# temudschin/xfemm

Hardware: AMD Instinct MI355X
Metric: solved DoF/s (assembly+CG to tol) on 2M-tri magnetostatic (higher is better)
Workload: dtype f64; 1 GPU; configs[2]: synthetic 2000000-tri square-domain magnetostatic, linear mu, tol 1e-08; triangles=2000000, dof_total=1002001, dof_per_gpu=1002001, nnz=7006001, pcg_iters=18, newton_iters=1, pcg=Chronopoulos-Gear + AMG V-cycle, parallelism=single GPU

## Files before the change

xfemm_amd/csrc/xfk_amg.h:

```cpp
#pragma once

#include <hip/hip_runtime.h>

#include <map>
#include <memory>
#include <vector>

#include "xfk_internal.h"
#include "xfk_partition.h"

struct xfk_comm;

namespace xfk {

constexpr int kAmgDenseMax = 2048;
constexpr int kAmgMaxLevels = 16;
constexpr int kAmgDeferSlots = 64;
constexpr int kAmgDeferTotal = kAmgDeferSlots + kAmgDeferSlots / 2;

struct AmgLevel {
    int n = 0;
    long long nnz = 0;
    int ncol_lim = 0;
    int ncol_smooth = 0;
// ... 156 lines not shown
    {
        if (side.cs) (void)hipStreamSynchronize(side.cs);
        if (sw.cs) (void)hipStreamSynchronize(sw.cs);
    }
    int setup(hipStream_t s, int n, int ncol_lim, const int *rowptr, const int *col, const double *val,
              long long nnz);
    int setup_dist(hipStream_t s, xfk_comm *comm, const HaloPlan &halo, int n, int nh, const int *rowptr,
                   const int *col, const double *val, long long nnz);
    int vcycle(hipStream_t s, const double *r, double *u, const int *done, double *part_gam = nullptr);
    bool gamma_done = false;
    int refresh(hipStream_t s, bool fold = true);
    int reserve_host();

  private:
    int init(hipStream_t s);
    int build(hipStream_t s, int l0);
    int aggregate(hipStream_t s, int l, long long &nc, bool allow_stop);
    int joins_and_p_impl(hipStream_t s, int l);
    int galerkin_dist(hipStream_t s, int l, int st, bool &rep);
    int fold_dist_tiles(hipStream_t s, int l);
    double *vc_dist(hipStream_t s, int l, const double *b, double *out, const int *done, int &rc);
    int host_ints(int count);
    int nd_order(hipStream_t s, const AmgLevel &C, int &ld);
    int resolve_deferred(hipStream_t s, bool &overflow);
    int fetch_deferred(hipStream_t s);
    int wait_deferred(hipStream_t s, bool &overflow);
    int dense_inverse(hipStream_t s, const AmgLevel &C, int ld);
    int alloc_vectors();
    int trace_strength(hipStream_t s, int l);
    int trace_aggregates(hipStream_t s, int l);
    long long ap_nnz = 0;
};

int amg_probe_info(Amg &M, hipStream_t s, xfk_amg_info *info);
int amg_probe_level_size(Amg &M, hipStream_t s, int level, int sel, int *rows, int *cols, long long *nnz);
int amg_probe_level_csr(Amg &M, hipStream_t s, int level, int sel, int *rowptr, int *col, double *val);
int amg_probe_tiles(Amg &M, hipStream_t s, int sel, int *tiles, int *wide);
int amg_probe_vector(Amg &M, hipStream_t s, int level, int what, double *out);
int amg_probe_trace(Amg &M, int level, int what, void *out);

}
```

xfemm_amd/csrc/xfk_amg.hip:

```cpp
#include <hipcub/hipcub.hpp>

#include <algorithm>
#include <climits>
#include <cmath>
#include <cstdio>
#include <cstdlib>
#include <cstring>
#include <map>
#include <mutex>
#include <vector>

#include "xfk_amg.h"
#include "xfk_comm.h"
#include "xfk_spmv.h"

namespace xfk {

namespace {


constexpr int kB = 256;
inline int nb(long long n) { return (int)((n + kB - 1) / kB); }

using MisKey = unsigned;
// ... 1014 lines not shown
    for (int s = 0; s < S; ++s) {
        bool lead = true;
#pragma unroll
        for (int q = 0; q <= s; ++q) lead = lead && !head[q];
        const double tot = lead ? cin + run[s] : run[s];
        h += head[s];
        const int nk = s + 1 < S ? key[s + 1] : __shfl_down(key[0], 1, G);
        const bool tail = key[s] != INT_MAX && (nk != key[s] || (s + 1 == S && l == G - 1));
        if (tail) {
            pcol[base + h - 1] = key[s];
            pval[base + h - 1] = tot;
        }
    }
    if (l == 0) cnt_out[row] = cnt;
}

template <int L>
__global__ void k_spgemm_compact(int nrows, int cap, const int *__restrict__ crow, const int *__restrict__ pcol,
                                 const double *__restrict__ pval, int *__restrict__ ccol, double *__restrict__ cval,
                                 int *nnz_out)
{
    const long long t = blockIdx.x * (long long)blockDim.x + threadIdx.x;
    if (t == 0 && nnz_out) *nnz_out = crow[nrows];
    const int row = (int)(t / L), l = (int)(t % L);
    if (row >= nrows) return;
    const int b = crow[row], n = crow[row + 1] - b;
    for (int m = l; m < n; m += L) {
        ccol[b + m] = pcol[(size_t)row * cap + m];
        cval[b + m] = pval[(size_t)row * cap + m];
    }
}

constexpr int kSlabLanes = 16;
__global__ void k_spgemm_compact_slab(int nrows, int nslab, int W, int stride, const int *__restrict__ crow,
                                      const int *__restrict__ slab_n, const int *__restrict__ pcol,
                                      const double *__restrict__ pval, int *__restrict__ ccol,
                                      double *__restrict__ cval, int *nnz_out)
{
    const long long t = blockIdx.x * (long long)blockDim.x + threadIdx.x;
    if (t == 0 && nnz_out) *nnz_out = crow[nrows];
    const int b = (int)(t / kSlabLanes), l = (int)(t % kSlabLanes);
    if (b >= nslab) return;
    const int d = crow[b * W], n = slab_n[b];
    const size_t src = (size_t)b * stride;
    for (int m = l; m < n; m += kSlabLanes) {
        ccol[d + m] = pcol[src + m];
        cval[d + m] = pval[src + m];
    }
}


constexpr int kBj = 64;

constexpr int kDsG = 16;
__global__ void k_dense_dscale(int n, int ld, const int *__restrict__ rowptr, const int *__restrict__ col,
                               const double *__restrict__ val, const int *__restrict__ iperm, double *__restrict__ sc)
{
    const int q = (blockIdx.x * blockDim.x + threadIdx.x) / kDsG, l = threadIdx.x % kDsG;
    if (q >= ld) return;
    const int i = iperm ? iperm[q] : (q < n ? q : -1);
    int kd = -1;
    if (i >= 0)
        for (int k = rowptr[i] + l; k < rowptr[i + 1]; k += kDsG)
            if (col[k] == i) kd = k;
#pragma unroll
    for (int off = 1; off < kDsG; off <<= 1) kd = max(kd, __shfl_xor(kd, off, kDsG));
    if (l != 0) return;
    const double d = kd >= 0 ? 0.0 + val[kd] : 0.0;
    sc[q] = d > 0.0 ? 1.0 / sqrt(d) : 1.0;
}
__global__ void k_dense_scatter(int n, int ld, const int *__restrict__ rowptr, const int *__restrict__ col,
                                const double *__restrict__ val, const int *__restrict__ perm,
                                const int *__restrict__ iperm, const double *__restrict__ sc, double *__restrict__ M)
{
    const int q = (blockIdx.x * blockDim.x + threadIdx.x) / kDsG, l = threadIdx.x % kDsG;
    if (q >= ld) return;
// ... 1139 lines not shown
    return XFK_OK;
}

int scan_only(DBuf<char> &tmp, hipStream_t s, const int *in, int *out, int n)
{
    if (n <= kScanLds) {
        k_scan_lds<<<1, 1024, 0, s>>>(n, in, out);
        AMG_CHECK(hipGetLastError());
        return XFK_OK;
    }
    size_t bytes = 0;
    AMG_CHECK(hipcub::DeviceScan::ExclusiveSum(nullptr, bytes, in, out, n + 1, s));
    AMG_CHECK(tmp.alloc(bytes ? bytes : 1));
    AMG_CHECK(hipcub::DeviceScan::ExclusiveSum(tmp.p, bytes, in, out, n + 1, s));
    return XFK_OK;
}
int scan_only(Amg &A, hipStream_t s, const int *in, int *out, int n) { return scan_only(A.cub_tmp, s, in, out, n); }

int read_flag(Amg &A, hipStream_t s, int idx, int &v)
{
    AMG_CHECK(hipMemcpyAsync(A.host_int + 1, A.dev_int.p + idx, sizeof(int), hipMemcpyDeviceToHost, s));
    AMG_CHECK(hipStreamSynchronize(s));
    v = A.host_int[1];
    return XFK_OK;
}

static bool spgemm_slab_on()
{
    return env_int("XFK_SPGEMM_SLAB", 1) != 0;
}

static int sort_rows_per_wave(int cap) { return cap == 16 ? 16 : cap <= 64 ? 8 : cap == 128 ? 4 : 2; }

void launch_compact(hipStream_t s, int nrows, int cap, const int *crow, const int *slab_n, const int *pc,
                    const double *pv, int *ccol, double *cval, int *nnz_out)
{
    if (slab_n) {
        const int W = sort_rows_per_wave(cap), nslab = (nrows + W - 1) / W;
        k_spgemm_compact_slab<<<(unsigned)(((long long)nslab * kSlabLanes + kB - 1) / kB), kB, 0, s>>>(
            nrows, nslab, W, W * cap, crow, slab_n, pc, pv, ccol, cval, nnz_out);
    } else if (cap <= 16)
        k_spgemm_compact<4><<<(unsigned)(((long long)nrows * 4 + kB - 1) / kB), kB, 0, s>>>(nrows, cap, crow, pc, pv,
                                                                                             ccol, cval, nnz_out);
    else if (cap <= 32)
        k_spgemm_compact<8><<<(unsigned)(((long long)nrows * 8 + kB - 1) / kB), kB, 0, s>>>(nrows, cap, crow, pc, pv,
                                                                                             ccol, cval, nnz_out);
    else
        k_spgemm_compact<16><<<(unsigned)(((long long)nrows * 16 + kB - 1) / kB), kB, 0, s>>>(nrows, cap, crow, pc,
                                                                                               pv, ccol, cval, nnz_out);
}

template <bool PMODE>
int spgemm(Amg &M, hipStream_t s, int nrows, const SgX &X, const SgY &Y, DBuf<int> &crow, DBuf<int> &ccol,
           DBuf<double> &cval, long long &cnnz, int key = -1, bool defer = true)
{
    AMG_CHECK(M.cnt.alloc((size_t)nrows + 1 + ((size_t)nrows + 1) / 2));
    AMG_CHECK(crow.alloc((size_t)nrows + 1));
    int *slab_n = spgemm_slab_on() ? M.cnt.p + nrows + 1 : nullptr;
    int *sovf = M.dev_int.p + 6;
    auto launch_sort = [&](int cap, int *ovf, int *need = nullptr) {
        int *pc = M.pad_col.p;
        double *pv = M.pad_val.p;
        if (nrows > 0) {
            if (cap == 16)
                k_spgemm_sort<PMODE, 4, 16><<<(nrows + 15) / 16, 64, 0, s>>>(nrows, X, Y, M.cnt.p, pc, pv, ovf, need,
                                                                             slab_n);
            else if (cap == 32)
                k_spgemm_sort<PMODE, 8, 32><<<(nrows + 7) / 8, 64, 0, s>>>(nrows, X, Y, M.cnt.p, pc, pv, ovf, need,
                                                                             slab_n);
            else if (cap == 64)
                k_spgemm_sort<PMODE, 8, 64><<<(nrows + 7) / 8, 64, 0, s>>>(nrows, X, Y, M.cnt.p, pc, pv, ovf, need,
                                                                             slab_n);
            else if (cap == 128)
                k_spgemm_sort<PMODE, 16, 128><<<(nrows + 3) / 4, 64, 0, s>>>(nrows, X, Y, M.cnt.p, pc, pv, ovf, need,
                                                                             slab_n);
            else
                k_spgemm_sort<PMODE, 32, 256><<<(nrows + 1) / 2, 64, 0, s>>>(nrows, X, Y, M.cnt.p, pc, pv, ovf, need,
                                                                             slab_n);
        }
    };
    auto sort_pass = [&](int cap, bool &overflow) -> int {
        AMG_CHECK(M.pad_col.alloc((size_t)nrows * cap));
        AMG_CHECK(M.pad_val.alloc((size_t)nrows * cap));
        AMG_CHECK(hipMemsetAsync(sovf, 0, sizeof(int), s));
        launch_sort(cap, sovf);
        AMG_CHECK(hipMemcpyAsync(M.host_int + 4, sovf, sizeof(int), hipMemcpyDeviceToHost, s));
        int rc = scan_total(M, s, M.cnt.p, crow.p, nrows, cnnz);
        if (rc != XFK_OK) return rc;
        overflow = M.host_int[4] != 0;
        if (overflow) return XFK_OK;
        AMG_CHECK(ccol.alloc((size_t)std::max(1LL, cnnz)));
        AMG_CHECK(cval.alloc((size_t)std::max(1LL, cnnz)));
        if (nrows > 0)
            launch_compact(s, nrows, cap, crow.p, slab_n, M.pad_col.p, M.pad_val.p, ccol.p, cval.p, nullptr);
        return XFK_OK;
    };
    auto deferred_pass = [&](int cap, bool verify = false) -> int {
        int *slot = M.def_dev.p + M.def_n;
        int *need = (verify && cap > 16) ? M.def_dev.p + kAmgDeferSlots + M.def_n / 2 : nullptr;
        M.def_verify[M.def_n / 2] = need ? cap : 0;
        AMG_CHECK(M.pad_col.alloc((size_t)nrows * cap));
        AMG_CHECK(M.pad_val.alloc((size_t)nrows * cap));
        AMG_CHECK(ccol.alloc((size_t)std::max(1LL, (long long)nrows * cap)));
        AMG_CHECK(cval.alloc((size_t)std::max(1LL, (long long)nrows * cap)));
        launch_sort(cap, slot, need);
        int rc = scan_only(M, s, M.cnt.p, crow.p, nrows);
        if (rc != XFK_OK) return rc;
        if (nrows > 0)
            launch_compact(s, nrows, cap, crow.p, slab_n, M.pad_col.p, M.pad_val.p, ccol.p, cval.p, slot + 1);
        else
            AMG_CHECK(hipMemsetAsync(slot + 1, 0, sizeof(int), s));
        M.def_target[M.def_n / 2] = &cnnz;
        M.def_n += 2;
        cnnz = (long long)nrows * cap;
        return XFK_OK;
    };
    if (key >= 0) {
        auto hint = M.cap_hint.find(key);
        if (hint != M.cap_hint.end()) {
            if (defer && M.def_n + 2 <= kAmgDeferSlots) return deferred_pass(hint->second, M.foreign);
            if (M.foreign) {
                M.cap_hint.erase(hint);
                hint = M.cap_hint.end();
            }
        }
        if (hint != M.cap_hint.end()) {
            bool overflow = false;
            int rc = sort_pass(hint->second, overflow);
            if (rc != XFK_OK || !overflow) return rc;
            M.cap_hint.erase(hint);
        }
    }
    int maxprod = 0;
    if (nrows > 0) {
        k_spgemm_nprod<PMODE><<<nb(nrows), kB, 0, s>>>(nrows, X, Y, M.cnt.p);
        size_t bytes = 0;
        AMG_CHECK(hipcub::DeviceReduce::Max(nullptr, bytes, M.cnt.p, M.dev_int.p + 3, nrows, s));
        AMG_CHECK(M.cub_tmp.alloc(bytes ? bytes : 1));
        AMG_CHECK(hipcub::DeviceReduce::Max(M.cub_tmp.p, bytes, M.cnt.p, M.dev_int.p + 3, nrows, s));
        int rc = read_flag(M, s, 3, maxprod);
        if (rc != XFK_OK) return rc;
    }
// ... 61 lines not shown
    const int g = (n + 255) / 256;
    if (G <= 4) {
        if (acc) k_csr_mv_tile<256, true, 2><<<g, 256, 0, s>>>(n, rowptr, col, val, x, y, done, c16, cbase);
        else k_csr_mv_tile<256, false, 2><<<g, 256, 0, s>>>(n, rowptr, col, val, x, y, done, c16, cbase);
    } else {
        if (acc) k_csr_mv_tile<256, true, 6><<<g, 256, 0, s>>>(n, rowptr, col, val, x, y, done, c16, cbase);
        else k_csr_mv_tile<256, false, 6><<<g, 256, 0, s>>>(n, rowptr, col, val, x, y, done, c16, cbase);
    }
}

void launch_mv(hipStream_t s, int n, const int *rowptr, const int *col, const double *val, const double *x, double *y,
               bool acc, int G, const int *done, const unsigned short *c16 = nullptr, const int *cbase = nullptr)
{
    if (n <= 0) return;
    if (n >= kTileMinRows && G <= 8) {
        const int g = (n + 255) / 256;
        if (G <= 4) {
            if (acc) k_csr_mv_tile<256, true, 2><<<g, 256, 0, s>>>(n, rowptr, col, val, x, y, done, c16, cbase);
            else k_csr_mv_tile<256, false, 2><<<g, 256, 0, s>>>(n, rowptr, col, val, x, y, done, c16, cbase);
        } else {
            if (acc) k_csr_mv_tile<256, true, 6><<<g, 256, 0, s>>>(n, rowptr, col, val, x, y, done, c16, cbase);
            else k_csr_mv_tile<256, false, 6><<<g, 256, 0, s>>>(n, rowptr, col, val, x, y, done, c16, cbase);
        }
        return;
    }
    const int g = (int)(((long long)n * G + 255) / 256);
#define XFK_MV(GG)                                                                                        \
    if (acc) k_csr_mv_g<GG, true><<<g, 256, 0, s>>>(n, rowptr, col, val, x, y, done);                    \
    else k_csr_mv_g<GG, false><<<g, 256, 0, s>>>(n, rowptr, col, val, x, y, done);
    if (G == 4) { XFK_MV(4) } else if (G == 8) { XFK_MV(8) } else { XFK_MV(16) }
#undef XFK_MV
}

}

__global__ void k_tile_halo_flags(int n, int B, const int *__restrict__ rowptr, const int *__restrict__ col,
                                  int *__restrict__ flag)
{
    const int i = blockIdx.x * blockDim.x + threadIdx.x;
    if (i >= n) return;
    bool h = false;
    for (int k = rowptr[i]; k < rowptr[i + 1]; ++k) h = h || col[k] >= n;
    if (h) flag[i / B] = 1;
}

int build_tile_split(hipStream_t s, int n, int B, const int *rowptr, const int *col, TileSplit &ts)
{
    const int nt = (n + B - 1) / B;
    ts.B = 0;
    ts.n_in = ts.n_bd = 0;
    if (nt == 0) {
        ts.B = B;
        return XFK_OK;
    }
    DBuf<int> flag;
    AMG_CHECK(flag.alloc(nt));
    AMG_CHECK(hipMemsetAsync(flag.p, 0, sizeof(int) * nt, s));
    k_tile_halo_flags<<<nb(n), kB, 0, s>>>(n, B, rowptr, col, flag.p);
    std::vector<int> h(nt), list;
    list.reserve(nt);
    AMG_CHECK(hipMemcpyAsync(h.data(), flag.p, sizeof(int) * nt, hipMemcpyDeviceToHost, s));
    AMG_CHECK(hipStreamSynchronize(s));
    for (int t = 0; t < nt; ++t)
        if (!h[t]) list.push_back(t);
    ts.n_in = (int)list.size();
    for (int t = 0; t < nt; ++t)
// ... 2103 lines not shown
```

xfemm_amd/csrc/xfk_api.hip:

```cpp
#include <hipcub/hipcub.hpp>

#include "xfk_amg.h"
#include "xfk_spmv.h"

#include <algorithm>
#include <atomic>
#include <chrono>
#include <cmath>
#include <cstring>
#include <map>
#include <mutex>
#include <iterator>
#include <set>
#include <type_traits>
#include <unordered_map>

#include "xfk_age.h"
#include "xfk_comm.h"
#include "xfk_kernels.h"
#include "xfk_magdir.h"
#include <cstdio>
#include <cstdlib>
#include "xfk_partition.h"

// ... 603 lines not shown

hipError_t d2h(void *dst, const void *src, size_t bytes, hipStream_t s)
{
    hipError_t e = hipMemcpyAsync(dst, src, bytes, hipMemcpyDeviceToHost, s);
    if (e != hipSuccess) return e;
    return hipStreamSynchronize(s);
}

static hipError_t cub_scratch(xfk_problem *P, size_t bytes, void **out)
{
    hipError_t e = P->cub_tmp.alloc(bytes ? bytes : 1);
    *out = P->cub_tmp.p;
    return e;
}

static hipError_t exclusive_scan(xfk_problem *P, const int *in, int *out, int n)
{
    hipStream_t s = P->stream;
    void *tmp = nullptr;
    size_t bytes = 0;
    hipError_t e = hipcub::DeviceScan::InclusiveSum(tmp, bytes, in, out + 1, n, s);
    if (e == hipSuccess) e = cub_scratch(P, bytes, &tmp);
    if (e == hipSuccess) e = hipMemsetAsync(out, 0, sizeof(int), s);
    if (e == hipSuccess) e = hipcub::DeviceScan::InclusiveSum(tmp, bytes, in, out + 1, n, s);
    return e;
}

static int alloc_cg(xfk_problem *P);

struct SymTmp {
    static constexpr int kMaxRounds = 4096;
    static constexpr int kMaxColors = 128;
    int *deg, *cursor, *cnt, *hist;
    int *rowcnt, *keys_out, *iota, *flag, *iperm, *rowtmp;
    unsigned char *active;
    unsigned long long *maxkey, *used;
    size_t zero_bytes = 0, bytes = 0;

    void carve(char *base, int N, int NE, int nfill)
    {
        size_t off = 0;
        auto take = [&](auto *&ptr, size_t n) {
            using T = std::remove_reference_t<decltype(*ptr)>;
            off = (off + 255) & ~size_t(255);
            ptr = base ? reinterpret_cast<T *>(base + off) : nullptr;
            off += (n ? n : 1) * sizeof(T);
        };
        take(deg, N);
        take(cursor, N);
        take(cnt, 4);
        take(hist, kMaxColors + 1);
        zero_bytes = off;
        take(rowcnt, N);
        take(active, N);
        take(keys_out, NE);
        take(iota, NE);
        take(flag, N);
        take(maxkey, N);
        take(used, 2 * (size_t)N);
        take(iperm, NE);
        take(rowtmp, (size_t)row_tmp_size(N, NE, nfill));
        bytes = off;
    }
};

int xfk_resolve_nnz(xfk_problem *P)
{
    if (!P->nnz_pending) return XFK_OK;
    XFK_CHECK(hipEventSynchronize(P->nnz_ev));
    P->nnz = P->hpin[0];
    P->nnz_own = P->hpin[1];
    P->row_max = P->hpin[5];
    P->nnz_pending = false;
    return XFK_OK;
}

int build_symbolic(xfk_problem *P)
{
    hipStream_t s = P->stream;
    P->ts.B = 0;
    const int N = P->NR, NL = P->NL, NE = P->NE;
    SymTmp T;
    std::vector<long long> fillv = P->pbc_fill;
    if (P->harmonic && P->ac_solver == 1) fillv.insert(fillv.end(), P->pbca_fill.begin(), P->pbca_fill.end());
    const int nfill = 2 * (int)fillv.size();
    T.carve(nullptr, NL, NE, nfill);
    XFK_CHECK(P->sym_tmp.alloc(T.bytes));
    T.carve(P->sym_tmp.p, NL, NE, nfill);
    XFK_CHECK(hipMemsetAsync(P->sym_tmp.p, 0, T.zero_bytes, s));

    XFK_CHECK(P->n2e_ptr.alloc(NL + 1));
    XFK_CHECK(P->n2e.alloc(3 * (size_t)NE));
    launch_n2e_count(s, NE, P->p_raw.p, T.deg);
    XFK_CHECK(exclusive_scan(P, T.deg, P->n2e_ptr.p, NL));
    launch_n2e_fill(s, NE, P->p_raw.p, P->n2e_ptr.p, T.cursor, P->n2e.p);
    launch_n2e_sort(s, N, NL, P->n2e_ptr.p, P->n2e.p);

    const int *fp = nullptr, *fc = nullptr;
    if (!fillv.empty()) {
        std::vector<std::vector<int>> rows(N);
        for (long long k : fillv) {
            int r = (int)(k >> 32), c = (int)(k & 0xffffffff);
            if (r < N) rows[r].push_back(c);
            if (c < N) rows[c].push_back(r);
        }
        std::vector<int> hptr(N + 1, 0), hcol;
        for (int r = 0; r < N; ++r) {
            std::sort(rows[r].begin(), rows[r].end());
            hptr[r + 1] = hptr[r] + (int)rows[r].size();
            hcol.insert(hcol.end(), rows[r].begin(), rows[r].end());
        }
        XFK_CHECK(upload(P->fill_ptr, hptr.data(), hptr.size(), s));
        XFK_CHECK(upload(P->fill_col, hcol.data(), hcol.size(), s));
        XFK_CHECK(hipStreamSynchronize(s));
        fp = P->fill_ptr.p;
        fc = P->fill_col.p;
    }

    XFK_CHECK(P->rowptr.alloc(N + 1));
    launch_row_build(s, N, P->p_raw.p, P->n2e_ptr.p, P->n2e.p, fp, fc, T.rowtmp, T.rowcnt, P->n2e.p);
    XFK_CHECK(exclusive_scan(P, T.rowcnt, P->rowptr.p, N));
    XFK_CHECK(hipMemcpyAsync(P->hpin, P->rowptr.p + N, sizeof(int), hipMemcpyDeviceToHost, s));
    XFK_CHECK(hipMemcpyAsync(P->hpin + 1, P->rowptr.p + P->N, sizeof(int), hipMemcpyDeviceToHost, s));
    P->hpin[5] = 0;
    if (!P->harmonic && N > 0 && P->amg && P->amg->cap_hint.empty()) {
        void *tmp = nullptr;
        size_t bytes = 0;
        XFK_CHECK(hipcub::DeviceReduce::Max(tmp, bytes, T.rowcnt, T.cnt + 3, N, s));
        XFK_CHECK(cub_scratch(P, bytes, &tmp));
        XFK_CHECK(hipcub::DeviceReduce::Max(tmp, bytes, T.rowcnt, T.cnt + 3, N, s));
        XFK_CHECK(hipMemcpyAsync(P->hpin + 5, T.cnt + 3, sizeof(int), hipMemcpyDeviceToHost, s));
    }
    const long long bound_nnz = 6LL * NE + N + nfill;
    const bool defer = !P->harmonic && P->age_key.empty() && P->pbc_entry_key.empty() &&
                       bound_nnz * 12 <= (512LL << 20);
    long long cap_nnz;
    if (defer) {
        if (!P->nnz_ev) XFK_CHECK(hipEventCreateWithFlags(&P->nnz_ev, hipEventDisableTiming));
        XFK_CHECK(hipEventRecord(P->nnz_ev, s));
        P->nnz_pending = true;
        cap_nnz = bound_nnz;
    } else {
        XFK_CHECK(hipStreamSynchronize(s));
        P->nnz = P->hpin[0];
        P->nnz_own = P->hpin[1];
        P->row_max = P->hpin[5];
        P->nnz_pending = false;
        cap_nnz = P->nnz;
    }
    XFK_CHECK(P->col.alloc(cap_nnz));
    XFK_CHECK(P->val.alloc(cap_nnz));
    XFK_CHECK(P->diag.alloc(N));
    launch_row_copy(s, N, P->p_raw.p, P->n2e_ptr.p, P->n2e.p, fp, fc, T.rowtmp, P->rowptr.p, P->col.p, P->diag.p);

    P->ncolors = 0;
    P->color_rounds = 0;
    if (P->harmonic) {
    XFK_CHECK(P->color.alloc(NE));
    XFK_CHECK(hipMemsetAsync(P->color.p, 0xff, sizeof(int) * NE, s));
    constexpr int kSyncRounds = 6;
    XFK_CHECK(hipMemsetAsync(T.active, 1, (size_t)NL, s));
    int round = 0, last = 0;
    for (;;) {
        XFK_REQUIRE(round < SymTmp::kMaxRounds, XFK_ERR_UNSUPPORTED, "element colouring did not terminate");
        for (int k = 0; k < kSyncRounds; ++k, ++round)
            launch_jp_round(s, NL, NE, round, T.active, T.cnt + 2, P->p_raw.p, P->n2e_ptr.p, P->n2e.p, P->color.p,
                            T.maxkey, T.used);
        XFK_CHECK(d2h(&last, T.cnt + 2, sizeof(int), s));
        if (last < round) break;
    }
    round = last + 1;
    P->color_rounds = round;
    const int maxc = SymTmp::kMaxColors;
    launch_color_hist(s, NE, P->color.p, T.hist, maxc);
    std::vector<int> hh(maxc + 1);
    XFK_CHECK(d2h(hh.data(), T.hist, sizeof(int) * (maxc + 1), s));
    XFK_REQUIRE(hh[maxc] == 0, XFK_ERR_UNSUPPORTED, "more than 128 element colours needed");
    int nc = 0;
    for (int c = 0; c < maxc; ++c)
        if (hh[c]) nc = c + 1;
    P->ncolors = nc;
    P->color_off.assign(nc + 1, 0);
    for (int c = 0; c < nc; ++c) P->color_off[c + 1] = P->color_off[c] + hh[c];

    XFK_CHECK(P->perm.alloc(NE));
    launch_iota(s, NE, T.iota);
// ... 2183 lines not shown
```

xfemm_amd/csrc/xfk_device.hip:

```cpp
#include "xfk_kernels.h"
#include "xfk_axi.h"
#include "xfk_spmv.h"

namespace xfk {


__device__ __forceinline__ double wave_sum(double v)
{
#pragma unroll
    for (int off = 32; off > 0; off >>= 1) v += __shfl_xor(v, off, 64);
    return v;
}

__device__ __forceinline__ double block_sum(double v, double *lds)
{
    v = wave_sum(v);
    const int lane = threadIdx.x & 63, wid = threadIdx.x >> 6;
    __syncthreads();
    if (lane == 0) lds[wid] = v;
    __syncthreads();
    double r = 0.0;
    if (threadIdx.x == 0) {
        const int nw = (blockDim.x + 63) >> 6;
        for (int w = 0; w < nw; ++w) r += lds[w];
// ... 168 lines not shown
    sort_node_list(ptr[v], ptr[v + 1], n2e);
}

__global__ void k_sort_segments(int N, const int *__restrict__ ptr, int *__restrict__ a)
{
    int v = blockIdx.x * blockDim.x + threadIdx.x;
    if (v >= N) return;
    int s = ptr[v], e = ptr[v + 1];
    for (int i = s + 1; i < e; ++i) {
        int key = a[i];
        int j = i - 1;
        while (j >= s && a[j] > key) {
            a[j + 1] = a[j];
            --j;
        }
        a[j + 1] = key;
    }
}

constexpr int kRowLds = 32;

struct RowCands {
    const int *p, *n2e_ptr, *n2e, *fill_ptr, *fill_col;
    __device__ __forceinline__ int count(int v) const
    {
        int ne = n2e_ptr[v + 1] - n2e_ptr[v];
        int nf = fill_ptr ? (fill_ptr[v + 1] - fill_ptr[v]) : 0;
        return 3 * ne + nf + 1;
    }
    __device__ __forceinline__ long long base(int v) const
    {
        return 3LL * n2e_ptr[v] + (fill_ptr ? fill_ptr[v] : 0) + v;
    }
};

constexpr int kRowRegElems = 15;

template <int W>
__device__ __forceinline__ void bitonic_regs(int (&a)[W])
{
#pragma unroll
    for (int k = 2; k <= W; k <<= 1)
#pragma unroll
        for (int j = k >> 1; j > 0; j >>= 1)
#pragma unroll
            for (int q = 0; q < W; ++q) {
                const int o = q ^ j;
                if (o > q) {
                    const bool up = (q & k) == 0;
                    const int x = a[q], y = a[o];
                    a[q] = up ? min(x, y) : max(x, y);
                    a[o] = up ? max(x, y) : min(x, y);
                }
            }
}

template <int W>
__device__ __forceinline__ void row_regs(int v, int s, int ne, const RowCands &rc, int (&a)[W])
{
    a[0] = v;
    int f[(W - 1) / 2];
#pragma unroll
    for (int q = 0; q < (W - 1) / 2; ++q) f[q] = q < ne ? rc.n2e[s + q] : -1;
#pragma unroll
    for (int q = 0; q < (W - 1) / 2; ++q) {
        int x = INT_MAX, y = INT_MAX, z = INT_MAX;
        if (f[q] >= 0) {
            x = rc.p[3 * f[q]];
            y = rc.p[3 * f[q] + 1];
            z = rc.p[3 * f[q] + 2];
        }
        a[1 + 2 * q] = x == v ? y : x;
        a[2 + 2 * q] = (x == v || y == v) ? z : y;
    }
#pragma unroll
    for (int q = 2 * ((W - 1) / 2) + 1; q < W; ++q) a[q] = INT_MAX;
    bitonic_regs(a);
}

__device__ __forceinline__ bool row_reg_ok(const RowCands &rc, int v, int ne)
{
    return ne <= kRowRegElems && !(rc.fill_ptr && rc.fill_ptr[v + 1] > rc.fill_ptr[v]);
}

template <int W>
__device__ __forceinline__ int row_regs_len(int v, int s, int ne, const RowCands &rc)
{
    int a[W];
    row_regs<W>(v, s, ne, rc, a);
    int u = 0;
#pragma unroll
    for (int q = 0; q < W; ++q) u += (a[q] != INT_MAX && (q == 0 || a[q] != a[q - 1])) ? 1 : 0;
    return u;
}

template <int W>
__device__ __forceinline__ void row_regs_write(int v, int s, int ne, const RowCands &rc, int r0,
                                               int *__restrict__ col, int *__restrict__ diag)
{
    int a[W];
    row_regs<W>(v, s, ne, rc, a);
    int u = 0;
#pragma unroll
    for (int q = 0; q < W; ++q)
        if (a[q] != INT_MAX && (q == 0 || a[q] != a[q - 1])) {
            col[r0 + u] = a[q];
            if (a[q] == v) diag[v] = r0 + u;
            ++u;
        }
}

__global__ void __launch_bounds__(kBlock) k_row_len_reg(int N, RowCands rc, int *__restrict__ tmp,
                                                        int *__restrict__ rowcnt, int *n2e_sort)
{
    __shared__ int s_c[kBlock * (kRowLds + 1)];
    const int v = blockIdx.x * kBlock + threadIdx.x;
    if (v >= N) return;
    const int s = rc.n2e_ptr[v], ne = rc.n2e_ptr[v + 1] - s;
    if (n2e_sort) sort_node_list(s, s + ne, n2e_sort);
    if (row_reg_ok(rc, v, ne)) {
        rowcnt[v] = ne <= 7 ? row_regs_len<16>(v, s, ne, rc) : row_regs_len<32>(v, s, ne, rc);
        return;
    }
    const int m = rc.count(v);
    int *out = tmp + rc.base(v);
    int *c = (m <= kRowLds) ? &s_c[threadIdx.x * (kRowLds + 1)] : out;
    int k = 0;
    for (int t = s; t < s + ne; ++t) {
        const int f = rc.n2e[t];
        c[k++] = rc.p[3 * f];
        c[k++] = rc.p[3 * f + 1];
        c[k++] = rc.p[3 * f + 2];
    }
    if (rc.fill_ptr)
        for (int t = rc.fill_ptr[v]; t < rc.fill_ptr[v + 1]; ++t) c[k++] = rc.fill_col[t];
    c[k++] = v;
    for (int i = 1; i < m; ++i) {
        const int key = c[i];
        int j = i - 1;
        while (j >= 0 && c[j] > key) {
            c[j + 1] = c[j];
            --j;
        }
        c[j + 1] = key;
    }
    int u = 0;
    for (int i = 0; i < m; ++i)
        if (u == 0 || c[i] != c[u - 1]) c[u++] = c[i];
    if (c != out)
        for (int i = 0; i < u; ++i) out[i] = c[i];
    rowcnt[v] = u;
}

__global__ void k_row_fill_reg(int N, RowCands rc, const int *__restrict__ tmp, const int *__restrict__ rowptr,
                               int *__restrict__ col, int *__restrict__ diag)
{
    const int v = blockIdx.x * blockDim.x + threadIdx.x;
    if (v >= N) return;
    const int s = rc.n2e_ptr[v], ne = rc.n2e_ptr[v + 1] - s;
    const int r0 = rowptr[v];
    if (row_reg_ok(rc, v, ne)) {
        if (ne <= 7) row_regs_write<16>(v, s, ne, rc, r0, col, diag);
        else row_regs_write<32>(v, s, ne, rc, r0, col, diag);
        return;
    }
    const int *src = tmp + rc.base(v);
    const int len = rowptr[v + 1] - r0;
    for (int i = 0; i < len; ++i) {
        const int c = src[i];
        col[r0 + i] = c;
        if (c == v) diag[v] = r0 + i;
    }
}

__device__ __forceinline__ unsigned hash_u32(unsigned x)
{
    x ^= x >> 16; x *= 0x7feb352dU;
    x ^= x >> 15; x *= 0x846ca68bU;
    x ^= x >> 16;
    return x;
}

__device__ __forceinline__ unsigned long long jp_key(int e)
{
    return ((unsigned long long)hash_u32((unsigned)e) << 32) | (unsigned)e;
}

__global__ void __launch_bounds__(kBlock) k_jp_nodes(int N, unsigned char *__restrict__ active,
                                                     const int *__restrict__ n2e_ptr, const int *__restrict__ n2e,
                                                     const int *__restrict__ color,
                                                     unsigned long long *__restrict__ maxkey,
                                                     unsigned long long *__restrict__ used)
{
    const int v = blockIdx.x * kBlock + threadIdx.x;
    if (v >= N || !active[v]) return;
    unsigned long long mk = 0, u0 = 0, u1 = 0;
    bool pending = false;
    const int t1 = n2e_ptr[v + 1];
    for (int t = n2e_ptr[v]; t < t1; ++t) {
        const int f = n2e[t];
        const int c = color[f];
        if (c < 0) {
            const unsigned long long k = jp_key(f);
            mk = k > mk ? k : mk;
// ... 711 lines not shown
static inline int nblk(long long n) { return (int)((n + kBlock - 1) / kBlock); }

int grid_reduce(int N)
{
    int t = (N + kBlock - 1) / kBlock;
    return t < kRedGrid ? (t > 0 ? t : 1) : kRedGrid;
}

void launch_count_incidence(hipStream_t s, int NE, const int *p, int *deg)
{
    if (NE) k_count_incidence<<<nblk(NE), kBlock, 0, s>>>(NE, p, deg);
}
void launch_fill_n2e(hipStream_t s, int NE, const int *p, const int *ptr, int *cursor, int *n2e)
{
    if (NE) k_fill_n2e<<<nblk(NE), kBlock, 0, s>>>(NE, p, ptr, cursor, n2e);
}
void launch_n2e_count(hipStream_t s, int NE, const int *p, int *deg)
{
    if (NE) k_n2e_tile<false><<<(NE + 255) / 256, 256, 0, s>>>(NE, p, nullptr, deg, nullptr);
}
void launch_n2e_fill(hipStream_t s, int NE, const int *p, const int *ptr, int *cursor, int *n2e)
{
    if (NE) k_n2e_tile<true><<<(NE + 255) / 256, 256, 0, s>>>(NE, p, ptr, cursor, n2e);
}
void launch_n2e_sort(hipStream_t s, int v0, int NL, const int *ptr, int *n2e)
{
    if (NL > v0) k_n2e_sort<<<nblk(NL - v0), kBlock, 0, s>>>(v0, NL, ptr, n2e);
}
void launch_sort_segments(hipStream_t s, int N, const int *ptr, int *a)
{
    if (N) k_sort_segments<<<nblk(N), kBlock, 0, s>>>(N, ptr, a);
}
long long row_tmp_size(int N, int NE, int nfill) { return 9LL * NE + nfill + N; }
void launch_row_build(hipStream_t s, int N, const int *p, const int *n2e_ptr, const int *n2e, const int *fill_ptr,
                      const int *fill_col, int *tmp, int *rowcnt, int *n2e_sort)
{
    RowCands rc{p, n2e_ptr, n2e, fill_ptr, fill_col};
    if (N) k_row_len_reg<<<nblk(N), kBlock, 0, s>>>(N, rc, tmp, rowcnt, n2e_sort);
}
void launch_row_copy(hipStream_t s, int N, const int *p, const int *n2e_ptr, const int *n2e, const int *fill_ptr,
                     const int *fill_col, const int *tmp, const int *rowptr, int *col, int *diag)
{
    RowCands rc{p, n2e_ptr, n2e, fill_ptr, fill_col};
    if (N) k_row_fill_reg<<<nblk(N), kBlock, 0, s>>>(N, rc, tmp, rowptr, col, diag);
}
void launch_jp_round(hipStream_t s, int N, int NE, int round, unsigned char *active, int *pending_round,
                     const int *p, const int *n2e_ptr, const int *n2e, int *color, unsigned long long *maxkey,
                     unsigned long long *used)
{
    if (N) k_jp_nodes<<<nblk(N), kBlock, 0, s>>>(N, active, n2e_ptr, n2e, color, maxkey, used);
    if (NE) k_jp_elems<<<nblk(NE), kBlock, 0, s>>>(NE, round, pending_round, p, maxkey, used, color);
}
void launch_color_hist(hipStream_t s, int NE, const int *color, int *hist, int maxc)
{
    if (NE) k_color_hist<<<std::min(nblk(NE), 2048), kBlock, 0, s>>>(NE, color, hist, maxc);
}
void launch_iota(hipStream_t s, int n, int *a)
{
    if (n) k_iota<<<nblk(n), kBlock, 0, s>>>(n, a);
}
void launch_build_erec(hipStream_t s, int NE, const int *perm, const int *p, const int *lbl, const int *ebits_raw,
                       int4 *erec, int *ebits, int *iperm)
{
    if (NE) k_build_erec<<<nblk(NE), kBlock, 0, s>>>(NE, perm, p, lbl, ebits_raw, erec, ebits, iperm);
}
void launch_build_slots(hipStream_t s, int NE, int nrows, const int *p, const int *iperm, const int *rowptr,
                        const int *col, int *slot, int *bad)
{
    if (NE) k_build_slots<<<nblk(NE), kBlock, 0, s>>>(NE, nrows, p, iperm, rowptr, col, slot, bad);
}
void launch_lookup_slots(hipStream_t s, int n, const int *rc, const int *rowptr, const int *col, int *out)
{
    if (n) k_lookup_slots<<<nblk(n), kBlock, 0, s>>>(n, rc, rowptr, col, out);
}
void launch_mark_fix_adj(hipStream_t s, int N, const int *rowptr, const int *col, const unsigned char *fixed,
                         int *flag)
{
// ... 79 lines not shown
```

xfemm_amd/csrc/xfk_kernels.h:

```cpp
#pragma once

#include "xfk_internal.h"

namespace xfk {

struct AssembleArgs {
    const int4 *erec;
    const int *ebits;
    const int *slot;
    const double *x, *y;
    const DevLabel *labels;
    const DevBlock *blocks;
    const DevLine *lines;
    const DevCirc *circs;
    const double *bhB, *bhH, *bhS;
    double *mu1, *mu2;
    const double *V;
    double *val, *b;
    int iter;
    int axi;
    double ext_ro, ext_ri, ext_zo;
    const int *p_raw, *lbl_raw, *ebits_raw, *n2e_ptr, *n2e, *rowptr, *col;
    double *mu1_out, *mu2_out;
    int *miss;
// ... 8 lines not shown
    const double *W, *dinv;
    double *Z, *P, *V, *R, *U;
    const double *gam_in;
    const double *del_in;
    const double *reso;
    double *gam_out;
    int Ggam, Gdel;
    CgState *S;
    long long it;
    int N;
    int amg;
};

int cg_grid(int N);
int cg_axpy_grid(int N);
void launch_cg_init_r(hipStream_t s, int N, int flag, const int *rowptr, const int *col, const double *val,
                      const double *b, double *V, double *R, double *U, double *Z, double *P, const double *dinv,
                      double *part_reso, double *part_gam0);
void launch_cg_axpy(hipStream_t s, const CgAxpyArgs &A);
void launch_cg_spmv(hipStream_t s, int N, const int *rowptr, const int *col, const double *val, const double *U,
                    double *W, double *part_del, const CgState *S, const double *R = nullptr,
                    double *part_gam = nullptr, const int *tiles = nullptr, int ntiles = 0,
                    const unsigned short *c16 = nullptr, const int *cbase = nullptr);
void launch_cg_dot(hipStream_t s, int N, const double *a, const double *b, double *part);
void launch_cg_state_init(hipStream_t s, CgState *S, double tol, double tol_rel = 0.0);

void launch_count_incidence(hipStream_t s, int NE, const int *p, int *deg);
void launch_fill_n2e(hipStream_t s, int NE, const int *p, const int *ptr, int *cursor, int *n2e);
void launch_sort_segments(hipStream_t s, int N, const int *ptr, int *a);
void launch_n2e_count(hipStream_t s, int NE, const int *p, int *deg);
void launch_n2e_fill(hipStream_t s, int NE, const int *p, const int *ptr, int *cursor, int *n2e);
void launch_n2e_sort(hipStream_t s, int v0, int NL, const int *ptr, int *n2e);
long long row_tmp_size(int N, int NE, int nfill);
void launch_row_build(hipStream_t s, int N, const int *p, const int *n2e_ptr, const int *n2e, const int *fill_ptr,
                      const int *fill_col, int *tmp, int *rowcnt,
                      int *n2e_sort = nullptr);
void launch_row_copy(hipStream_t s, int N, const int *p, const int *n2e_ptr, const int *n2e, const int *fill_ptr,
                     const int *fill_col, const int *tmp, const int *rowptr, int *col, int *diag);
void launch_jp_round(hipStream_t s, int N, int NE, int round, unsigned char *active, int *pending_round,
                     const int *p, const int *n2e_ptr, const int *n2e, int *color, unsigned long long *maxkey,
                     unsigned long long *used);
void launch_color_hist(hipStream_t s, int NE, const int *color, int *hist, int maxc);
void launch_iota(hipStream_t s, int n, int *a);
void launch_build_erec(hipStream_t s, int NE, const int *perm, const int *p, const int *lbl, const int *ebits_raw,
                       int4 *erec, int *ebits, int *iperm);
void launch_build_slots(hipStream_t s, int NE, int nrows, const int *p, const int *iperm, const int *rowptr,
                        const int *col, int *slot, int *bad);
void launch_add_at_slots(hipStream_t s, int n, const int *slot, const double *v, double *data);
void launch_lookup_slots(hipStream_t s, int n, const int *rc, const int *rowptr, const int *col, int *out);
void launch_mark_fix_adj(hipStream_t s, int N, const int *rowptr, const int *col, const unsigned char *fixed,
                         int *flag);
void launch_compact_flags(hipStream_t s, int N, const int *flag, int *cursor, int *out);
void launch_assemble_rows(hipStream_t s, int N, const AssembleArgs &A);
void launch_point_currents(hipStream_t s, int n, const int *nodes, const double *J, double *b);
void launch_dirichlet(hipStream_t s, int nrows, const int *rows, int nadj, const int *nadj_dev, int nadj_max,
                      const int *adj, const int *rowptr, const int *col, const int *diag, const unsigned char *fixed,
                      const double *fix_first, const double *fix_last, double *val, double *b);
void launch_map(hipStream_t s, int n, const int *dst, const int *ptr, const int *src, const double *w,
                double *data, double *tmp);
void launch_diag_inv(hipStream_t s, int N, const int *diag, const double *val, double *dinv, CgState *S);
void launch_newton_res(hipStream_t s, int N, const double *V, const double *Vold, double *partials,
                       unsigned *counter, NewtonScalars *S);
void launch_relax(hipStream_t s, int N, double relax, double *V, const double *Vold);
void launch_scale(hipStream_t s, int N, double sc, const double *V, double *out);

}
```

Baseline: 188.0 million DoF/s.

## Build CSR pattern in one slab pass and scan per-slab counts

```diff
diff --git a/xfemm_amd/csrc/xfk_amg.h b/xfemm_amd/csrc/xfk_amg.h
--- a/xfemm_amd/csrc/xfk_amg.h
+++ b/xfemm_amd/csrc/xfk_amg.h
@@ -212,6 +212,8 @@
     long long ap_nnz = 0;
 };
 
+int scan_offsets(DBuf<char> &tmp, hipStream_t s, const int *in, int *out, int n);
+
 int amg_probe_info(Amg &M, hipStream_t s, xfk_amg_info *info);
 int amg_probe_level_size(Amg &M, hipStream_t s, int level, int sel, int *rows, int *cols, long long *nnz);
 int amg_probe_level_csr(Amg &M, hipStream_t s, int level, int sel, int *rowptr, int *col, double *val);
diff --git a/xfemm_amd/csrc/xfk_amg.hip b/xfemm_amd/csrc/xfk_amg.hip
--- a/xfemm_amd/csrc/xfk_amg.hip
+++ b/xfemm_amd/csrc/xfk_amg.hip
@@ -1070,16 +1070,31 @@
 }
 
 constexpr int kSlabLanes = 16;
-__global__ void k_spgemm_compact_slab(int nrows, int nslab, int W, int stride, const int *__restrict__ crow,
-                                      const int *__restrict__ slab_n, const int *__restrict__ pcol,
-                                      const double *__restrict__ pval, int *__restrict__ ccol,
-                                      double *__restrict__ cval, int *nnz_out)
+__global__ void k_spgemm_compact_slab(int nrows, int nslab, int W, int stride, const int *__restrict__ sbase,
+                                      const int *__restrict__ cnt, const int *__restrict__ pcol,
+                                      const double *__restrict__ pval, int *__restrict__ crow,
+                                      int *__restrict__ ccol, double *__restrict__ cval, int *nnz_out)
 {
     const long long t = blockIdx.x * (long long)blockDim.x + threadIdx.x;
-    if (t == 0 && nnz_out) *nnz_out = crow[nrows];
+    if (t == 0) {
+        crow[nrows] = sbase[nslab];
+        if (nnz_out) *nnz_out = sbase[nslab];
+    }
     const int b = (int)(t / kSlabLanes), l = (int)(t % kSlabLanes);
     if (b >= nslab) return;
-    const int d = crow[b * W], n = slab_n[b];
+    const int d = sbase[b], n = sbase[b + 1] - d;
+    {
+        const int row = b * W + l;
+        const bool has = l < W && row < nrows;
+        const int c = has ? cnt[row] : 0;
+        int upto = c;
+#pragma unroll
+        for (int off = 1; off < kSlabLanes; off <<= 1) {
+            const int o = __shfl_up(upto, off, kSlabLanes);
+            if (l >= off) upto += o;
+        }
+        if (has) crow[row] = d + upto - c;
+    }
     const size_t src = (size_t)b * stride;
     for (int m = l; m < n; m += kSlabLanes) {
         ccol[d + m] = pcol[src + m];
@@ -2285,13 +2300,13 @@
 
 static int sort_rows_per_wave(int cap) { return cap == 16 ? 16 : cap <= 64 ? 8 : cap == 128 ? 4 : 2; }
 
-void launch_compact(hipStream_t s, int nrows, int cap, const int *crow, const int *slab_n, const int *pc,
+void launch_compact(hipStream_t s, int nrows, int cap, int *crow, const int *sbase, const int *cnt, const int *pc,
                     const double *pv, int *ccol, double *cval, int *nnz_out)
 {
-    if (slab_n) {
+    if (sbase) {
         const int W = sort_rows_per_wave(cap), nslab = (nrows + W - 1) / W;
         k_spgemm_compact_slab<<<(unsigned)(((long long)nslab * kSlabLanes + kB - 1) / kB), kB, 0, s>>>(
-            nrows, nslab, W, W * cap, crow, slab_n, pc, pv, ccol, cval, nnz_out);
+            nrows, nslab, W, W * cap, sbase, cnt, pc, pv, crow, ccol, cval, nnz_out);
     } else if (cap <= 16)
         k_spgemm_compact<4><<<(unsigned)(((long long)nrows * 4 + kB - 1) / kB), kB, 0, s>>>(nrows, cap, crow, pc, pv,
                                                                                              ccol, cval, nnz_out);
@@ -2307,9 +2322,13 @@
 int spgemm(Amg &M, hipStream_t s, int nrows, const SgX &X, const SgY &Y, DBuf<int> &crow, DBuf<int> &ccol,
            DBuf<double> &cval, long long &cnnz, int key = -1, bool defer = true)
 {
-    AMG_CHECK(M.cnt.alloc((size_t)nrows + 1 + ((size_t)nrows + 1) / 2));
+    const size_t cnt_len = ((size_t)nrows + 4) & ~size_t(3), slab_len = (((size_t)nrows + 1) / 2 + 5) & ~size_t(3);
+    AMG_CHECK(M.cnt.alloc(cnt_len + 2 * slab_len));
     AMG_CHECK(crow.alloc((size_t)nrows + 1));
-    int *slab_n = spgemm_slab_on() ? M.cnt.p + nrows + 1 : nullptr;
+    const bool slab = spgemm_slab_on() && nrows > 0;
+    int *slab_n = slab ? M.cnt.p + cnt_len : nullptr;
+    int *sbase = slab ? slab_n + slab_len : nullptr;
+    auto nslab_of = [&](int cap) { const int W = sort_rows_per_wave(cap); return (nrows + W - 1) / W; };
     int *sovf = M.dev_int.p + 6;
     auto launch_sort = [&](int cap, int *ovf, int *need = nullptr) {
         int *pc = M.pad_col.p;
@@ -2338,14 +2357,15 @@
         AMG_CHECK(hipMemsetAsync(sovf, 0, sizeof(int), s));
         launch_sort(cap, sovf);
         AMG_CHECK(hipMemcpyAsync(M.host_int + 4, sovf, sizeof(int), hipMemcpyDeviceToHost, s));
-        int rc = scan_total(M, s, M.cnt.p, crow.p, nrows, cnnz);
+        int rc = slab ? scan_total(M, s, slab_n, sbase, nslab_of(cap), cnnz)
+                      : scan_total(M, s, M.cnt.p, crow.p, nrows, cnnz);
         if (rc != XFK_OK) return rc;
         overflow = M.host_int[4] != 0;
         if (overflow) return XFK_OK;
         AMG_CHECK(ccol.alloc((size_t)std::max(1LL, cnnz)));
         AMG_CHECK(cval.alloc((size_t)std::max(1LL, cnnz)));
         if (nrows > 0)
-            launch_compact(s, nrows, cap, crow.p, slab_n, M.pad_col.p, M.pad_val.p, ccol.p, cval.p, nullptr);
+            launch_compact(s, nrows, cap, crow.p, sbase, M.cnt.p, M.pad_col.p, M.pad_val.p, ccol.p, cval.p, nullptr);
         return XFK_OK;
     };
     auto deferred_pass = [&](int cap, bool verify = false) -> int {
@@ -2357,10 +2377,11 @@
         AMG_CHECK(ccol.alloc((size_t)std::max(1LL, (long long)nrows * cap)));
         AMG_CHECK(cval.alloc((size_t)std::max(1LL, (long long)nrows * cap)));
         launch_sort(cap, slot, need);
-        int rc = scan_only(M, s, M.cnt.p, crow.p, nrows);
+        int rc = slab ? scan_only(M, s, slab_n, sbase, nslab_of(cap)) : scan_only(M, s, M.cnt.p, crow.p, nrows);
         if (rc != XFK_OK) return rc;
         if (nrows > 0)
-            launch_compact(s, nrows, cap, crow.p, slab_n, M.pad_col.p, M.pad_val.p, ccol.p, cval.p, slot + 1);
+            launch_compact(s, nrows, cap, crow.p, sbase, M.cnt.p, M.pad_col.p, M.pad_val.p, ccol.p, cval.p,
+                           slot + 1);
         else
             AMG_CHECK(hipMemsetAsync(slot + 1, 0, sizeof(int), s));
         M.def_target[M.def_n / 2] = &cnnz;
@@ -2488,6 +2509,11 @@
 #undef XFK_MV
 }
 
+}
+
+int scan_offsets(DBuf<char> &tmp, hipStream_t s, const int *in, int *out, int n)
+{
+    return scan_only(tmp, s, in, out, n);
 }
 
 __global__ void k_tile_halo_flags(int n, int B, const int *__restrict__ rowptr, const int *__restrict__ col,
diff --git a/xfemm_amd/csrc/xfk_api.hip b/xfemm_amd/csrc/xfk_api.hip
--- a/xfemm_amd/csrc/xfk_api.hip
+++ b/xfemm_amd/csrc/xfk_api.hip
@@ -659,7 +659,7 @@
     static constexpr int kMaxRounds = 4096;
     static constexpr int kMaxColors = 128;
     int *deg, *cursor, *cnt, *hist;
-    int *rowcnt, *keys_out, *iota, *flag, *iperm, *rowtmp;
+    int *rowcnt, *keys_out, *iota, *flag, *iperm, *rowtmp, *rowslab, *slab_n, *sbase;
     unsigned char *active;
     unsigned long long *maxkey, *used;
     size_t zero_bytes = 0, bytes = 0;
@@ -687,6 +687,9 @@
         take(used, 2 * (size_t)N);
         take(iperm, NE);
         take(rowtmp, (size_t)row_tmp_size(N, NE, nfill));
+        take(rowslab, (size_t)row_slab_size(N, NE, nfill));
+        take(slab_n, (size_t)(N + 63) / 64 + 1);
+        take(sbase, (size_t)(N + 63) / 64 + 1);
         bytes = off;
     }
 };
@@ -745,8 +748,26 @@
     }
 
     XFK_CHECK(P->rowptr.alloc(N + 1));
-    launch_row_build(s, N, P->p_raw.p, P->n2e_ptr.p, P->n2e.p, fp, fc, T.rowtmp, T.rowcnt, P->n2e.p);
-    XFK_CHECK(exclusive_scan(P, T.rowcnt, P->rowptr.p, N));
+    XFK_CHECK(P->diag.alloc(N));
+    const int nslab = (N + 63) / 64;
+    launch_row_slab(s, N, P->p_raw.p, P->n2e_ptr.p, P->n2e.p, fp, fc, T.rowtmp, T.rowslab, T.rowcnt, T.slab_n,
+                    P->diag.p, P->n2e.p);
+    {
+        const int rc = scan_offsets(P->cub_tmp, s, T.slab_n, T.sbase, nslab);
+        if (rc != XFK_OK) return rc;
+    }
+    const long long bound_nnz = 6LL * NE + N + nfill;
+    const bool defer = !P->harmonic && P->age_key.empty() && P->pbc_entry_key.empty() &&
+                       bound_nnz * 12 <= (512LL << 20);
+    if (N == 0) XFK_CHECK(hipMemsetAsync(P->rowptr.p, 0, sizeof(int), s));
+    if (defer) {
+        XFK_CHECK(P->col.alloc(bound_nnz));
+        launch_row_compact(s, N, P->n2e_ptr.p, fp, T.sbase, T.rowcnt, T.rowslab, P->rowptr.p, P->col.p, P->diag.p,
+                           true, true);
+    } else {
+        launch_row_compact(s, N, P->n2e_ptr.p, fp, T.sbase, T.rowcnt, T.rowslab, P->rowptr.p, nullptr, P->diag.p,
+                           true, false);
+    }
     XFK_CHECK(hipMemcpyAsync(P->hpin, P->rowptr.p + N, sizeof(int), hipMemcpyDeviceToHost, s));
     XFK_CHECK(hipMemcpyAsync(P->hpin + 1, P->rowptr.p + P->N, sizeof(int), hipMemcpyDeviceToHost, s));
     P->hpin[5] = 0;
@@ -758,9 +779,6 @@
         XFK_CHECK(hipcub::DeviceReduce::Max(tmp, bytes, T.rowcnt, T.cnt + 3, N, s));
         XFK_CHECK(hipMemcpyAsync(P->hpin + 5, T.cnt + 3, sizeof(int), hipMemcpyDeviceToHost, s));
     }
-    const long long bound_nnz = 6LL * NE + N + nfill;
-    const bool defer = !P->harmonic && P->age_key.empty() && P->pbc_entry_key.empty() &&
-                       bound_nnz * 12 <= (512LL << 20);
     long long cap_nnz;
     if (defer) {
         if (!P->nnz_ev) XFK_CHECK(hipEventCreateWithFlags(&P->nnz_ev, hipEventDisableTiming));
@@ -777,8 +795,9 @@
     }
     XFK_CHECK(P->col.alloc(cap_nnz));
     XFK_CHECK(P->val.alloc(cap_nnz));
-    XFK_CHECK(P->diag.alloc(N));
-    launch_row_copy(s, N, P->p_raw.p, P->n2e_ptr.p, P->n2e.p, fp, fc, T.rowtmp, P->rowptr.p, P->col.p, P->diag.p);
+    if (!defer)
+        launch_row_compact(s, N, P->n2e_ptr.p, fp, T.sbase, T.rowcnt, T.rowslab, P->rowptr.p, P->col.p, P->diag.p,
+                           false, true);
 
     P->ncolors = 0;
     P->color_rounds = 0;
diff --git a/xfemm_amd/csrc/xfk_device.hip b/xfemm_amd/csrc/xfk_device.hip
--- a/xfemm_amd/csrc/xfk_device.hip
+++ b/xfemm_amd/csrc/xfk_device.hip
@@ -224,6 +224,10 @@
     {
         return 3LL * n2e_ptr[v] + (fill_ptr ? fill_ptr[v] : 0) + v;
     }
+    __device__ __forceinline__ long long slab(int v0) const
+    {
+        return 2LL * n2e_ptr[v0] + (fill_ptr ? fill_ptr[v0] : 0) + v0;
+    }
 };
 
 constexpr int kRowRegElems = 15;
@@ -275,93 +279,120 @@
     return ne <= kRowRegElems && !(rc.fill_ptr && rc.fill_ptr[v + 1] > rc.fill_ptr[v]);
 }
 
-template <int W>
-__device__ __forceinline__ int row_regs_len(int v, int s, int ne, const RowCands &rc)
-{
-    int a[W];
-    row_regs<W>(v, s, ne, rc, a);
+__global__ void __launch_bounds__(kBlock) k_row_slab(int N, RowCands rc, int *__restrict__ tmp,
+                                                     int *__restrict__ slab, int *__restrict__ rowcnt,
+                                                     int *__restrict__ slab_n, int *__restrict__ dloc, int *n2e_sort)
+{
+    __shared__ int s_c[kBlock * (kRowLds + 1)];
+    const int v = blockIdx.x * kBlock + threadIdx.x, lane = threadIdx.x & 63;
+    if (v - lane >= N) return;
+    const bool live = v < N;
+    int a[32];
+    const int *c = nullptr;
     int u = 0;
-#pragma unroll
-    for (int q = 0; q < W; ++q) u += (a[q] != INT_MAX && (q == 0 || a[q] != a[q - 1])) ? 1 : 0;
-    return u;
-}
-
-template <int W>
-__device__ __forceinline__ void row_regs_write(int v, int s, int ne, const RowCands &rc, int r0,
-                                               int *__restrict__ col, int *__restrict__ diag)
-{
-    int a[W];
-    row_regs<W>(v, s, ne, rc, a);
-    int u = 0;
-#pragma unroll
-    for (int q = 0; q < W; ++q)
+    long long sb = 0;
+    if (live) {
+        const int s = rc.n2e_ptr[v], ne = rc.n2e_ptr[v + 1] - s;
+        if (n2e_sort) sort_node_list(s, s + ne, n2e_sort);
+        if (lane == 0) sb = rc.slab(v);
+        if (row_reg_ok(rc, v, ne)) {
+            if (ne <= 7) {
+                int h[16];
+                row_regs<16>(v, s, ne, rc, h);
+#pragma unroll
+                for (int q = 0; q < 16; ++q) {
+                    a[q] = h[q];
+                    a[16 + q] = INT_MAX;
+                }
+            } else {
+                row_regs<32>(v, s, ne, rc, a);
+            }
+#pragma unroll
+            for (int q = 0; q < 32; ++q) u += (a[q] != INT_MAX && (q == 0 || a[q] != a[q - 1])) ? 1 : 0;
+        } else {
+            const int m = rc.count(v);
+            int *w = (m <= kRowLds) ? &s_c[threadIdx.x * (kRowLds + 1)] : tmp + rc.base(v);
+            int k = 0;
+            for (int t = s; t < s + ne; ++t) {
+                const int f = rc.n2e[t];
+                w[k++] = rc.p[3 * f];
+                w[k++] = rc.p[3 * f + 1];
+                w[k++] = rc.p[3 * f + 2];
+            }
+            if (rc.fill_ptr)
+                for (int t = rc.fill_ptr[v]; t < rc.fill_ptr[v + 1]; ++t) w[k++] = rc.fill_col[t];
+            w[k++] = v;
+            for (int i = 1; i < m; ++i) {
+                const int key = w[i];
+                int j = i - 1;
+                while (j >= 0 && w[j] > key) {
+                    w[j + 1] = w[j];
+                    --j;
+                }
+                w[j + 1] = key;
+            }
+            for (int i = 0; i < m; ++i)
+                if (u == 0 || w[i] != w[u - 1]) w[u++] = w[i];
+            c = w;
+        }
+    }
+    int upto = u;
+#pragma unroll
+    for (int off = 1; off < 64; off <<= 1) {
+        const int t = __shfl_up(upto, off, 64);
+        if (lane >= off) upto += t;
+    }
+    if (lane == 63) slab_n[v >> 6] = upto;
+    sb = __shfl(sb, 0, 64);
+    if (!live) return;
+    rowcnt[v] = u;
+    int *dst = slab + sb + (upto - u);
+    if (c) {
+        for (int i = 0; i < u; ++i) {
+            const int x = c[i];
+            dst[i] = x;
+            if (x == v) dloc[v] = i;
+        }
+        return;
+    }
+    int k = 0;
+#pragma unroll
+    for (int q = 0; q < 32; ++q)
         if (a[q] != INT_MAX && (q == 0 || a[q] != a[q - 1])) {
-            col[r0 + u] = a[q];
-            if (a[q] == v) diag[v] = r0 + u;
-            ++u;
-        }
-}
-
-__global__ void __launch_bounds__(kBlock) k_row_len_reg(int N, RowCands rc, int *__restrict__ tmp,
-                                                        int *__restrict__ rowcnt, int *n2e_sort)
-{
-    __shared__ int s_c[kBlock * (kRowLds + 1)];
-    const int v = blockIdx.x * kBlock + threadIdx.x;
-    if (v >= N) return;
-    const int s = rc.n2e_ptr[v], ne = rc.n2e_ptr[v + 1] - s;
-    if (n2e_sort) sort_node_list(s, s + ne, n2e_sort);
-    if (row_reg_ok(rc, v, ne)) {
-        rowcnt[v] = ne <= 7 ? row_regs_len<16>(v, s, ne, rc) : row_regs_len<32>(v, s, ne, rc);
-        return;
-    }
-    const int m = rc.count(v);
-    int *out = tmp + rc.base(v);
-    int *c = (m <= kRowLds) ? &s_c[threadIdx.x * (kRowLds + 1)] : out;
-    int k = 0;
-    for (int t = s; t < s + ne; ++t) {
-        const int f = rc.n2e[t];
-        c[k++] = rc.p[3 * f];
-        c[k++] = rc.p[3 * f + 1];
-        c[k++] = rc.p[3 * f + 2];
-    }
-    if (rc.fill_ptr)
-        for (int t = rc.fill_ptr[v]; t < rc.fill_ptr[v + 1]; ++t) c[k++] = rc.fill_col[t];
-    c[k++] = v;
-    for (int i = 1; i < m; ++i) {
-        const int key = c[i];
-        int j = i - 1;
-        while (j >= 0 && c[j] > key) {
-            c[j + 1] = c[j];
-            --j;
-        }
-        c[j + 1] = key;
-    }
-    int u = 0;
-    for (int i = 0; i < m; ++i)
-        if (u == 0 || c[i] != c[u - 1]) c[u++] = c[i];
-    if (c != out)
-        for (int i = 0; i < u; ++i) out[i] = c[i];
-    rowcnt[v] = u;
-}
-
-__global__ void k_row_fill_reg(int N, RowCands rc, const int *__restrict__ tmp, const int *__restrict__ rowptr,
-                               int *__restrict__ col, int *__restrict__ diag)
-{
-    const int v = blockIdx.x * blockDim.x + threadIdx.x;
-    if (v >= N) return;
-    const int s = rc.n2e_ptr[v], ne = rc.n2e_ptr[v + 1] - s;
-    const int r0 = rowptr[v];
-    if (row_reg_ok(rc, v, ne)) {
-        if (ne <= 7) row_regs_write<16>(v, s, ne, rc, r0, col, diag);
-        else row_regs_write<32>(v, s, ne, rc, r0, col, diag);
-        return;
-    }
-    const int *src = tmp + rc.base(v);
-    const int len = rowptr[v + 1] - r0;
-    for (int i = 0; i < len; ++i) {
-        const int c = src[i];
-        col[r0 + i] = c;
-        if (c == v) diag[v] = r0 + i;
+            dst[k] = a[q];
+            if (a[q] == v) dloc[v] = k;
+            ++k;
+        }
+}
+
+template <bool PTRS, bool COPY>
+__global__ void __launch_bounds__(kBlock) k_row_compact(int N, int nslab, RowCands rc, const int *__restrict__ sbase,
+                                                        const int *__restrict__ rowcnt, const int *__restrict__ slab,
+                                                        int *__restrict__ rowptr, int *__restrict__ col,
+                                                        int *__restrict__ diag)
+{
+    const int b = blockIdx.x * (kBlock / 64) + threadIdx.x / 64, lane = threadIdx.x & 63;
+    if (b >= nslab) return;
+    const int d = sbase[b];
+    if (PTRS) {
+        if (b == 0 && lane == 0) rowptr[N] = sbase[nslab];
+        const int v = 64 * b + lane;
+        const int n = v < N ? rowcnt[v] : 0;
+        int upto = n;
+#pragma unroll
+        for (int off = 1; off < 64; off <<= 1) {
+            const int t = __shfl_up(upto, off, 64);
+            if (lane >= off) upto += t;
+        }
+        if (v < N) {
+            rowptr[v] = d + upto - n;
+            diag[v] += d + upto - n;
+        }
+    }
+    if (COPY) {
+        const int n = sbase[b + 1] - d;
+        const int *src = slab + rc.slab(64 * b);
+        for (int m = lane; m < n; m += 64) col[d + m] = src[m];
     }
 }
 
@@ -1139,17 +1170,25 @@
     if (N) k_sort_segments<<<nblk(N), kBlock, 0, s>>>(N, ptr, a);
 }
 long long row_tmp_size(int N, int NE, int nfill) { return 9LL * NE + nfill + N; }
-void launch_row_build(hipStream_t s, int N, const int *p, const int *n2e_ptr, const int *n2e, const int *fill_ptr,
-                      const int *fill_col, int *tmp, int *rowcnt, int *n2e_sort)
+long long row_slab_size(int N, int NE, int nfill) { return 6LL * NE + nfill + N; }
+void launch_row_slab(hipStream_t s, int N, const int *p, const int *n2e_ptr, const int *n2e, const int *fill_ptr,
+                     const int *fill_col, int *tmp, int *slab, int *rowcnt, int *slab_n, int *dloc, int *n2e_sort)
 {
     RowCands rc{p, n2e_ptr, n2e, fill_ptr, fill_col};
-    if (N) k_row_len_reg<<<nblk(N), kBlock, 0, s>>>(N, rc, tmp, rowcnt, n2e_sort);
-}
-void launch_row_copy(hipStream_t s, int N, const int *p, const int *n2e_ptr, const int *n2e, const int *fill_ptr,
-                     const int *fill_col, const int *tmp, const int *rowptr, int *col, int *diag)
-{
-    RowCands rc{p, n2e_ptr, n2e, fill_ptr, fill_col};
-    if (N) k_row_fill_reg<<<nblk(N), kBlock, 0, s>>>(N, rc, tmp, rowptr, col, diag);
+    if (N) k_row_slab<<<nblk(N), kBlock, 0, s>>>(N, rc, tmp, slab, rowcnt, slab_n, dloc, n2e_sort);
+}
+void launch_row_compact(hipStream_t s, int N, const int *n2e_ptr, const int *fill_ptr, const int *sbase,
+                        const int *rowcnt, const int *slab, int *rowptr, int *col, int *diag, bool ptrs, bool copy)
+{
+    if (!N) return;
+    RowCands rc{nullptr, n2e_ptr, nullptr, fill_ptr, nullptr};
+    const int nslab = (N + 63) / 64, g = (nslab + kBlock / 64 - 1) / (kBlock / 64);
+#define XFK_RC(PTRS, COPY) \
+    k_row_compact<PTRS, COPY><<<g, kBlock, 0, s>>>(N, nslab, rc, sbase, rowcnt, slab, rowptr, col, diag)
+    if (ptrs && copy) XFK_RC(true, true);
+    else if (ptrs) XFK_RC(true, false);
+    else if (copy) XFK_RC(false, true);
+#undef XFK_RC
 }
 void launch_jp_round(hipStream_t s, int N, int NE, int round, unsigned char *active, int *pending_round,
                      const int *p, const int *n2e_ptr, const int *n2e, int *color, unsigned long long *maxkey,
diff --git a/xfemm_amd/csrc/xfk_kernels.h b/xfemm_amd/csrc/xfk_kernels.h
--- a/xfemm_amd/csrc/xfk_kernels.h
+++ b/xfemm_amd/csrc/xfk_kernels.h
@@ -64,11 +64,12 @@
 void launch_n2e_fill(hipStream_t s, int NE, const int *p, const int *ptr, int *cursor, int *n2e);
 void launch_n2e_sort(hipStream_t s, int v0, int NL, const int *ptr, int *n2e);
 long long row_tmp_size(int N, int NE, int nfill);
-void launch_row_build(hipStream_t s, int N, const int *p, const int *n2e_ptr, const int *n2e, const int *fill_ptr,
-                      const int *fill_col, int *tmp, int *rowcnt,
-                      int *n2e_sort = nullptr);
-void launch_row_copy(hipStream_t s, int N, const int *p, const int *n2e_ptr, const int *n2e, const int *fill_ptr,
-                     const int *fill_col, const int *tmp, const int *rowptr, int *col, int *diag);
+long long row_slab_size(int N, int NE, int nfill);
+void launch_row_slab(hipStream_t s, int N, const int *p, const int *n2e_ptr, const int *n2e, const int *fill_ptr,
+                     const int *fill_col, int *tmp, int *slab, int *rowcnt, int *slab_n, int *dloc,
+                     int *n2e_sort = nullptr);
+void launch_row_compact(hipStream_t s, int N, const int *n2e_ptr, const int *fill_ptr, const int *sbase,
+                        const int *rowcnt, const int *slab, int *rowptr, int *col, int *diag, bool ptrs, bool copy);
 void launch_jp_round(hipStream_t s, int N, int NE, int round, unsigned char *active, int *pending_round,
                      const int *p, const int *n2e_ptr, const int *n2e, int *color, unsigned long long *maxkey,
                      unsigned long long *used);
```

Result: no change. 187.7 million DoF/s (median of 2 runs) (-0.1%).
